# OverLordGoldDragon/ssqueezepy

Measured on AMD Instinct MI355X. Metric: ssq_cwt transforms/sec (N=160k, 300 scales, f32), higher is better.
Workload: dtype f32; 1 GPU; ssq_cwt('gmw'), N=160000, 300 log scales (nv=32), float32, two-chirp+noise; algo=blockzoom+tiles, tile_kernel=float64 tile, unordered ds_add_f64, column pair per lane (tile3_kernel)

## Files before the change

### ssqueezepy_amd/csrc/ssq_blocks.h

```cpp
#pragma once
#include "ssq_common.h"
#include "ssq_fft.h"
#include "ssq_tiles.h"
#include <algorithm>
#include <vector>

namespace ssq {

struct BlockRowDev {
    int32_t cls;
    int32_t klo;
    int32_t KP;
    int32_t L;
    int32_t G;
    int32_t pb_off;
};

struct BlockClassDev {
    int64_t P, m, V, nb;
    int64_t ctw_off;
    int64_t xb_off;
    int64_t blk_off;
    int64_t xb_stride;
    int64_t analytic;
};

struct BlockPlan {
    int64_t M = 0, N = 0, n1 = 0, na = 0, max_batch = 1;
    int dtype = SSQ_F32;
    int group = 1;
    int ncu = 256;
    int nc = 0;
    DeviceArena mem;
    std::vector<BlockClassDev> hcls;
    BlockClassDev* classes = nullptr;
    BlockRowDev* rows = nullptr;
    void* pbank = nullptr;
    void* pxi = nullptr;
    void* ctw = nullptr; void* ftw = nullptr;
    void* items[5] = {nullptr, nullptr, nullptr, nullptr, nullptr};
    std::vector<int32_t> h_items[5];
    int64_t n_items[5] = {0, 0, 0, 0, 0};
    int64_t ftw_off[5] = {0, 0, 0, 0, 0};
    void* blocks = nullptr;
    void* xb = nullptr;
    std::vector<FftPlan> ffts;
    std::vector<int> fft_first;
    void* xa = nullptr;
    FftPlan inv_m;
    AnalyticFft* ana = nullptr;
    int n_analytic = 0;
    bool own4096 = false;
    bool own_big = false;
    int64_t n_generic = 0;
    bool exact_ok = false;
    int exA = 0, exB = 0, n_exact = 0;
    void* twM = nullptr; void* zbuf = nullptr;
    const float* e_bank = nullptr; const int64_t* e_off = nullptr; const int32_t* e_lo = nullptr;
    const int32_t* e_rows = nullptr;
    int setup_exact(const float* bank_dev, const int64_t* band_off_dev, const int32_t* band_lo_dev,
                    const int32_t* gen_rows_dev, const std::vector<int64_t>& h_off,
                    const std::vector<int32_t>& h_lo, const std::vector<int32_t>& h_gen);
    int run_exact(int sig, int nsig, const void* xh_all, float* Wx, float* dWx, float* w, unsigned short* kidx,
                  const float* row_scale, double dt, const SsqParams& sp, hipStream_t stream);

    int create(const ssq_cwt_blocks_desc& d, int dtype, int64_t M, int64_t N, int64_t n1, int64_t na,
               int64_t max_batch);
    void destroy();
    int64_t bytes() const;
    int spectra(const void* xp, const void* xh, int64_t batch, hipStream_t stream,
                const unsigned char* need = nullptr);
    int run(int sig, int nsig, float* Wx, float* dWx, float* w, unsigned short* kidx,
            const float* row_scale, double dt, const SsqParams& sp, hipStream_t stream,
            const int64_t* limit = nullptr);
    int run64(int sig, int nsig, double* Wx, double* dWx, double* w, unsigned short* kidx,
              const double* row_scale, double dt, const SsqParams& sp, hipStream_t stream);
};

}
```

### ssqueezepy_amd/csrc/ssq_cwt_blocks.hip

```cpp
#include "ssq_common.h"
#include "ssq_blocks.h"
#include "ssq_ldsfft.h"
#include <cmath>

namespace ssq {

#include "ssq_point_math.inl"

struct EmitRow {
    float2* W; float2* D; float* w; unsigned short* k;
    float rs; bool scale; double gamma; int64_t omax;
    float m2hi, m2lo;
    int fx, fa;
};
__device__ __forceinline__ EmitRow make_emit_row(float* Wx, float* dWx, float* w, unsigned short* kidx,
                                                 const float* row_scale, int sig, int ksig, int row,
                                                 int64_t na, int64_t N, double gamma, int flipud) {
    EmitRow e;
    const int64_t base = ((int64_t)sig * na + row) * N;
    e.W = reinterpret_cast<float2*>(Wx) + base;
    e.D = dWx ? reinterpret_cast<float2*>(dWx) + base : nullptr;
    e.w = w ? w + base : nullptr;
    e.k = kidx ? kidx + (int64_t)ksig * na * N + kidx_index(row, 0, na, N) : nullptr;
    e.scale = row_scale != nullptr;
// ... 2 lines not shown
    const float g2 = (float)(gamma * gamma);
    e.m2hi = g2 * 1.000004f; e.m2lo = g2 * 0.999996f;
    e.fx = flipud ? -1 : 0; e.fa = flipud ? (int)na : 0;
    return e;
}
template <bool LEAN, int GRID>
__device__ __forceinline__ bool emit_point(const EmitRow& e, int j, c32 W, c32 D, const SsqParams& sp) {
    float c = W.x, d = W.y, a = D.x, b = D.y;
    if constexpr (LEAN) {
        e.W[(unsigned)j] = make_float2(c, d);
        const float m2 = c * c + d * d, num = b * c - a * d;
        const bool above = m2 > e.m2hi, below = m2 < e.m2lo;
        const float w32 = fabsf(num * __builtin_amdgcn_rcpf(m2 * 6.2831855f));
        bool ok;
        const int kb = bin_screen_cwt<GRID>(w32, sp, (int)e.omax, ok);
        const int kf = (kb ^ e.fx) + e.fa;
        e.k[(unsigned)j] = (unsigned short)(above ? kf : 0xFFFF);
        return !(below | (above & ok));
    } else {
        c = c * e.rs; d = d * e.rs; a = a * e.rs; b = b * e.rs;
        e.W[j] = make_float2(c, d);
        if (e.D) e.D[j] = make_float2(a, b);
        if (e.w) {
            float wv;
            if (mag_lt(c, d, (float)e.gamma)) wv = INFINITY;
            else wv = (float)fabs(phase_ratio(a, b, c, d));
            e.w[j] = wv;
        }
        if (e.k) {
            const int above = mag_gt_screen(c, d, e.gamma);
            if (above < 0) return true;
            unsigned short kk = 0xFFFFu;
            if (above) {
                const int kb = bin_of_point_screen(a, b, c, d, sp, (int)e.omax);
                if (kb == -2) return true;
                kk = (unsigned short)(sp.flipud ? (int)e.omax - kb : kb);
            }
            e.k[j] = kk;
        }
        return false;
    }
}
template <int V> struct GridTag { static constexpr int value = V; };
template <bool LEAN, typename F>
__device__ __forceinline__ void dispatch_grid(int grid, F&& f) {
    if constexpr (LEAN) {
        if (grid == SSQ_GRID_LOG) f(GridTag<SSQ_GRID_LOG>{});
        else if (grid == SSQ_GRID_LOG_PIECEWISE) f(GridTag<SSQ_GRID_LOG_PIECEWISE>{});
        else f(GridTag<SSQ_GRID_LIN>{});
    } else {
        f(GridTag<-1>{});
    }
}
__device__ __forceinline__ void emit_point_exact(const EmitRow& e, unsigned short* kout, c32 W, c32 D,
                                                 const SsqParams& sp) {
    const float c = W.x * e.rs, d = W.y * e.rs, a = D.x * e.rs, b = D.y * e.rs;
    unsigned short kk = 0xFFFFu;
    if (mag_of(c, d) > e.gamma) {
        const int64_t kb = bin_of_point_exact(a, b, c, d, sp, e.omax);
        kk = (unsigned short)(sp.flipud ? e.omax - kb : kb);
    }
    *kout = kk;
}
struct BlockArgs {
    const int4* items;
    const BlockRowDev* rows;
    const BlockClassDev* classes;
    const float* pbank;
    const float* pxi;
    const c32* ctw;
    const c32* ftw;
    const c32* xb;
    const float* row_scale;
    float* Wx; float* dWx; float* w; unsigned short* kidx;
    int64_t M, N, na, n_items;
    double h;
    float inv_dt;
    double gamma;
    int sig;
    bool lean() const { return kidx && !dWx && !w && !row_scale; }
    bool wx_alone() const { return !kidx && !dWx && !w; }
};

template <int L, bool LEAN, bool NOD = false>
__device__ __forceinline__ void blockzoom_body(const BlockArgs& A, const SsqParams& sp, int item_idx,
                                               c32* __restrict__ buf, c32* __restrict__ spow,
                                               c32* __restrict__ wrapf, c32* __restrict__ bandW,
                                               c32* __restrict__ bandD) {
    using S = FftShape<L>;
    constexpr int G = S::G, R1 = S::R1, RL = S::RL;
    const int tid = threadIdx.x;
    const int4 item = A.items[item_idx];
    const int row = item.x, blk = item.y, c0 = item.z;
    const BlockRowDev r = A.rows[row];
    const BlockClassDev cl = A.classes[item.w];
    const int P = (int)cl.P, Rp = P / L;
    const int sig = A.sig + (int)blockIdx.y;
    const c32* xb = A.xb + cl.xb_off + ((int64_t)sig * cl.nb + blk) * cl.xb_stride;
    const c32* ctw = A.ctw + cl.ctw_off;
    const float* psi = A.pbank + r.pb_off;
    const float* pxi = A.pxi + r.pb_off;

    constexpr bool STAGE = (L <= 512);
    const float invP = 1.0f / (float)P;
    constexpr bool EARLY = !STAGE && (R1 * G <= NT);
    float e_p[EARLY ? PPT : 1], e_m[EARLY ? PPT : 1];
    c32 e_X[EARLY ? PPT : 1], e_cw[EARLY ? PPT / R1 : 1];
    if constexpr (EARLY) {
        constexpr int NBe = PPT / R1, STR = L / R1;
        c32 st_v = {0.f, 0.f}, st_w = {0.f, 0.f};
        if (tid < R1 * G) {
            const unsigned t = (unsigned)(tid / G), col = (unsigned)(c0 + tid % G);
            st_v = ctw[(t * (unsigned)STR * col) & (unsigned)(P - 1)];
        }
        if (tid < G) st_w = ctw[(0u - (unsigned)L * (unsigned)(c0 + tid)) & (unsigned)(P - 1)];
#pragma unroll
        for (int it = 0; it < NBe; ++it) {
            const int idx = tid + it * NT, g = idx % G, u = idx / G;
            const int off0 = (u - r.klo) & (L - 1);
            e_cw[it] = ctw[((unsigned)(r.klo + off0) * (unsigned)(c0 + g)) & (unsigned)(P - 1)];
#pragma unroll
            for (int k = 0; k < R1; ++k) {
                const int off = (off0 + k * STR) & (L - 1);
                const bool in = off < r.KP;
                e_p[it * R1 + k] = in ? psi[off] : 0.f;
                e_X[it * R1 + k] = in ? xb[r.klo + off] : c32{0.f, 0.f};
                e_m[it * R1 + k] = in ? pxi[off] : 0.f;
            }
        }
        if (tid < R1 * G) spow[tid] = st_v;
        if (tid < G) wrapf[tid] = st_w;
    } else {
        constexpr int STR = L / R1;
        for (int i = tid; i < R1 * G; i += NT) {
            const unsigned t = (unsigned)(i / G), col = (unsigned)(c0 + i % G);
            spow[i] = ctw[(t * (unsigned)STR * col) & (unsigned)(P - 1)];
        }
        if (tid < G) {
            const unsigned col = (unsigned)(c0 + tid);
            wrapf[tid] = ctw[(0u - (unsigned)L * col) & (unsigned)(P - 1)];
        }
        if constexpr (STAGE) {
            for (int off = tid; off < L; off += NT) {
                c32 b = {0.f, 0.f}, d = {0.f, 0.f};
                if (off < r.KP) {
                    const float p = psi[off] * invP;
                    const c32 X = xb[r.klo + off];
                    b = {p * X.x, p * X.y};
                    const float mm = pxi[off] * A.inv_dt;
                    d = {-(b.y * mm), b.x * mm};
                }
                bandW[off] = b; bandD[off] = d;
            }
        }
    }
    __syncthreads();
    c32 zw[PPT], zd[PPT];
    {
        constexpr int NB = PPT / R1, STR = L / R1;
#pragma unroll
        for (int it = 0; it < NB; ++it) {
            const int idx = tid + it * NT, g = idx % G, u = idx / G;
            const unsigned col = (unsigned)(c0 + g);
            const int off0 = (u - r.klo) & (L - 1);
            const c32 cw0 = EARLY ? e_cw[EARLY ? it : 0] : ctw[((unsigned)(r.klo + off0) * col) & (unsigned)(P - 1)];
            const c32 wf = wrapf[g];
#pragma unroll
            for (int k = 0; k < R1; ++k) {
                const int offu = off0 + k * STR;
                const int off = offu & (L - 1);
                c32 z = {0.f, 0.f}, dz = {0.f, 0.f};
                if constexpr (STAGE) {
                    c32 cw = (k == 0) ? cw0 : cmul_v(cw0, spow[k * G + g]);
                    if (offu >= L) cw = cmul_v(cw, wf);
                    z = cmul_v(bandW[off], cw);
                    dz = cmul_v(bandD[off], cw);
                } else if (EARLY || off < r.KP) {
                    const float p = (EARLY ? e_p[EARLY ? it * R1 + k : 0] : psi[off]) * invP;
                    const c32 X = EARLY ? e_X[EARLY ? it * R1 + k : 0] : xb[r.klo + off];
                    c32 cw = (k == 0) ? cw0 : cmul_v(cw0, spow[k * G + g]);
                    if (offu >= L) cw = cmul_v(cw, wf);
                    const c32 bz = {p * X.x, p * X.y};
                    z = cmul_v(bz, cw);
                    const float mm = (EARLY ? e_m[EARLY ? it * R1 + k : 0] : pxi[off]) * A.inv_dt;
                    dz = {-(z.y * mm), z.x * mm};
                }
                zw[it * R1 + k] = z; zd[it * R1 + k] = dz;
            }
        }
    }
    lds_ifft<L, true, true>(zw, buf, A.ftw, tid);
    if constexpr (!NOD) lds_ifft<L, true>(zd, buf, A.ftw, tid);

    constexpr int NB = PPT / RL, STR = L / RL;
    const EmitRow er = make_emit_row(A.Wx, A.dWx, A.w, A.kidx, A.row_scale, sig, (int)blockIdx.y, row, A.na, A.N, A.gamma, sp.flipud);
    const int m = (int)cl.m, N = (int)A.N;
    const int jbase = blk * (int)cl.V - m + c0;
    const unsigned span = (unsigned)max(0, min((int)cl.V, N - blk * (int)cl.V));
    unsigned pend = 0;
    auto emit_all = [&](auto grid_tag) {
        constexpr int GRID = decltype(grid_tag)::value;
#pragma unroll
        for (int it = 0; it < NB; ++it) {
            const int idx = tid + it * NT, g = idx % G, u = idx / G;
#pragma unroll
            for (int k = 0; k < RL; ++k) {
                const int dcol = (u + k * STR) * Rp + g + (c0 - m);
                if ((unsigned)dcol >= span) continue;
                const int j = dcol + blk * (int)cl.V;
                if constexpr (NOD) {
                    er.W[j] = make_float2(zw[it * RL + k].x * er.rs, zw[it * RL + k].y * er.rs);
                    continue;
                }
                if (emit_point<LEAN, GRID>(er, j, zw[it * RL + k], NOD ? c32{0.f, 0.f} : zd[it * RL + k], sp))
                    pend |= 1u << (it * RL + k);
            }
        }
    };
    dispatch_grid<LEAN>(sp.grid, emit_all);
    while (__builtin_amdgcn_ballot_w64(pend != 0)) {
        const unsigned low = pend & (0u - pend);
        pend ^= low;
        c32 W = {0.f, 0.f}, D = {0.f, 0.f};
        int j = 0;
#pragma unroll
        for (int it = 0; it < NB; ++it) {
            const int idx = tid + it * NT, g = idx % G, u = idx / G;
#pragma unroll
            for (int k = 0; k < RL; ++k)
                if (low == (1u << (it * RL + k))) {
                    W = zw[it * RL + k]; D = NOD ? c32{0.f, 0.f} : zd[it * RL + k]; j = jbase + (u + k * STR) * Rp + g;
                }
        }
        if (low) emit_point_exact(er, er.k + j, W, D, sp);
    }
}

template <int L, bool LEAN, bool NOD = false>
__global__ __launch_bounds__(NT) void blockzoom_kernel(BlockArgs A, SsqParams sp) {
    __shared__ c32 buf[D_POINTS];
    __shared__ c32 spow[FftShape<L>::R1 * FftShape<L>::G];
    __shared__ c32 wrapf[FftShape<L>::G];
    __shared__ c32 bandW[(L <= 512) ? L : 1], bandD[(L <= 512) ? L : 1];
    blockzoom_body<L, LEAN, NOD>(A, sp, (int)blockIdx.x, buf, spow, wrapf, bandW, bandD);
}

struct BlockMultiArgs {
    BlockArgs A;
    const int4* items[5]; const c32* ftw[5];
    int first[6];
};
template <bool LEAN, bool NOD = false>
__global__ __launch_bounds__(NT) void blockzoom_multi_kernel(BlockMultiArgs M, SsqParams sp) {
    __shared__ c32 buf[D_POINTS];
    __shared__ c32 spow[512];
    __shared__ c32 wrapf[32];
    __shared__ c32 bandW[512], bandD[512];
    const int b = (int)blockIdx.x;
    int s = 0;
#pragma unroll
    for (int k = 1; k < 5; ++k) s += b >= M.first[k];
    BlockArgs A = M.A;
    A.items = M.items[s]; A.ftw = M.ftw[s];
    const int it = b - M.first[s];
    switch (s) {
        case 0: blockzoom_body<128, LEAN, NOD>(A, sp, it, buf, spow, wrapf, bandW, bandD); break;
        case 1: blockzoom_body<256, LEAN, NOD>(A, sp, it, buf, spow, wrapf, bandW, bandD); break;
        case 2: blockzoom_body<512, LEAN, NOD>(A, sp, it, buf, spow, wrapf, bandW, bandD); break;
        case 3: blockzoom_body<1024, LEAN, NOD>(A, sp, it, buf, spow, wrapf, bandW, bandD); break;
        default: blockzoom_body<2048, LEAN, NOD>(A, sp, it, buf, spow, wrapf, bandW, bandD); break;
    }
}

struct BlockArgs64 {
    const int4* items; const BlockRowDev* rows; const BlockClassDev* classes;
    const double* pbank; const double* pxi;
    const c64* ctw; const c64* ftw; const c64* xb;
    const double* row_scale;
    double* Wx; double* dWx; double* w; unsigned short* kidx;
    int64_t M, N, na, n_items;
    double inv_dt, gamma;
    int sig;
    bool wx_alone() const { return !kidx && !dWx && !w; }
};

template <int L, bool NOD = false>
__global__ __launch_bounds__(FftGeom<double>::NT) SSQ_WAVES_PER_EU(2, 2) void blockzoom_f64_kernel(BlockArgs64 A, SsqParams sp) {
    using S = FftShape<L, double>;
    constexpr int NT64 = FftGeom<double>::NT, G = S::G, R1 = S::R1, RL = S::RL;
    __shared__ c64 buf[FftGeom<double>::D];
    __shared__ c64 spow[R1 * G];
    __shared__ c64 wrapf[G];
    const int tid = threadIdx.x;
    const int4 item = A.items[blockIdx.x];
    const int row = item.x, blk = item.y, c0 = item.z;
    const BlockRowDev r = A.rows[row];
    const BlockClassDev cl = A.classes[item.w];
    const int P = (int)cl.P, Rp = P / L;
    const int sig = A.sig + (int)blockIdx.y;
    const c64* xb = A.xb + cl.xb_off + ((int64_t)sig * cl.nb + blk) * cl.xb_stride;
    const c64* ctw = A.ctw + cl.ctw_off;
    const double* psi = A.pbank + r.pb_off;
    const double* pxi = A.pxi + r.pb_off;
    const double invP = 1.0 / (double)P;
    constexpr int NBP = PPT / R1, STRP = L / R1;
    double bp[PPT], bm[PPT]; c64 bX[PPT];
#pragma unroll
    for (int it = 0; it < NBP; ++it) {
        const int u = (tid + it * NT64) / G;
        const int off0 = (u - r.klo) & (L - 1);
#pragma unroll
        for (int k = 0; k < R1; ++k) {
            const int off = (off0 + k * STRP) & (L - 1);
            const int oc = off < r.KP ? off : 0;
            bp[it * R1 + k] = psi[oc]; bX[it * R1 + k] = xb[r.klo + oc]; bm[it * R1 + k] = pxi[oc];
        }
    }
    {
        constexpr int STR = L / R1;
        for (int i = tid; i < R1 * G; i += NT64) {
            const unsigned t = (unsigned)(i / G), col = (unsigned)(c0 + i % G);
            spow[i] = ctw[(t * (unsigned)STR * col) & (unsigned)(P - 1)];
        }
        if (tid < G) {
            const unsigned col = (unsigned)(c0 + tid);
            wrapf[tid] = ctw[(0u - (unsigned)L * col) & (unsigned)(P - 1)];
        }
    }
    c64 cw0s[NBP];
#pragma unroll
    for (int it = 0; it < NBP; ++it) {
        const int idx = tid + it * NT64, g = idx % G, u = idx / G;
        const int off0 = (u - r.klo) & (L - 1);
        cw0s[it] = ctw[((unsigned)(r.klo + off0) * (unsigned)(c0 + g)) & (unsigned)(P - 1)];
    }
    __syncthreads();
    c64 zw[PPT], zd[PPT];
    {
        constexpr int NB = PPT / R1, STR = L / R1;
#pragma unroll
        for (int it = 0; it < NB; ++it) {
            const int idx = tid + it * NT64, g = idx % G, u = idx / G;
            const int off0 = (u - r.klo) & (L - 1);
            const c64 cw0 = cw0s[it];
            const c64 wf = wrapf[g];
#pragma unroll
            for (int k = 0; k < R1; ++k) {
                const int offu = off0 + k * STR, off = offu & (L - 1);
                const bool in = off < r.KP;
                const double p = bp[it * R1 + k] * invP;
                const c64 X = bX[it * R1 + k];
                const double mm = bm[it * R1 + k] * A.inv_dt;
                c64 cw = (k == 0) ? cw0 : cmul(cw0, spow[k * G + g]);
// ... 365 lines not shown
                                                   c32* __restrict__ stw) {
    constexpr int L = WIDE_L, P = L * C, NTH = 64 * CW, SL = CW / C;
    const int tid = threadIdx.x;
    const int g = tid % CW, u = tid / CW, slot = g / C, r = g % C;
    const int64_t sig = blockIdx.y, M = A.M;
    const bool ana = k.analytic != 0;
    const int nunits = ana ? (int)k.nb : ((int)k.nb + 1) / 2;
    const c32* __restrict__ tw = A.ctw + k.ctw_off;
    const c32* __restrict__ xa = A.xa + sig * M;
    const float* __restrict__ xp = A.xp + sig * M;
    const int64_t lead = A.n1 - k.m;
    const int m32 = (int)M;
    wide_stage_tw<CW, C>(stw, tw, tid);
    c32 w[PPT / C][C];
    wide_load_w<CW, C>(w, tw, tid);
    c32 z[PPT];
    {
        const int unit = b * SL + slot;
        const bool live = unit < nunits;
        const int b0 = ana ? unit : 2 * unit, b1 = b0 + 1;
        const bool two = !ana && b1 < (int)k.nb;
        int64_t o0 = (lead + (int64_t)b0 * k.V) % M; if (o0 < 0) o0 += M;
        int64_t o1 = (lead + (int64_t)b1 * k.V) % M; if (o1 < 0) o1 += M;
        const int a0 = (int)o0, a1 = (int)o1;
#pragma unroll
        for (int t = 0; t < PPT; ++t) {
            const int p = (u + t * (L / 16)) * C + r;
            int s0 = a0 + p; if (s0 >= m32) s0 -= m32;
            int s1 = a1 + p; if (s1 >= m32) s1 -= m32;
            c32 v = {0.f, 0.f};
            if (live) {
                if (ana) v = xa[s0];
                else v = {xp[s0], two ? xp[s1] : 0.f};
            }
            z[t] = v;
        }
    }
    wide_ifft<CW>(z, buf, stw, tid);
    wide_natural<CW, C>(z, buf, w, tid);
    for (int sl = 0; sl < SL; ++sl) {
        const int unit = b * SL + sl;
        if (unit >= nunits) break;
        const int b0 = ana ? unit : 2 * unit;
        const bool two = !ana && b0 + 1 < (int)k.nb;
        const c32* __restrict__ Y = buf + sl * P;
        c32* out0 = A.xb + k.xb_off + (sig * k.nb + b0) * k.xb_stride;
        if (ana) {
            for (int f = tid; f < P; f += NTH) out0[f] = Y[(P - f) & (P - 1)];
        } else {
            c32* out1 = out0 + k.xb_stride;
            for (int f = tid; f <= P / 2; f += NTH) {
                const c32 Pk = Y[f], Qk = Y[(P - f) & (P - 1)];
                out0[f] = {0.5f * (Qk.x + Pk.x), 0.5f * (Qk.y - Pk.y)};
                if (two) out1[f] = {0.5f * (Qk.y + Pk.y), 0.5f * (Pk.x - Qk.x)};
            }
        }
    }
}
template <int QMAX>
__global__ __launch_bounds__(NT * QMAX) void block_spectra_multi_kernel(BlockSpecArgs A) {
    __shared__ c32 buf[4096 * QMAX];
    __shared__ c32 stw[WIDE_L];
    int b = (int)blockIdx.x, c = 0;
    while (c + 1 < A.ncls && b >= A.first[c + 1]) ++c;
    b -= A.first[c];
    const BlockClassDev k = A.classes[A.cls[c]];
    if (k.P == A.M && k.nb == 1 && !k.analytic && A.xh) {
        const int64_t M = A.M, sig = blockIdx.y;
        int64_t o = (A.n1 - k.m) % M; if (o < 0) o += M;
        const c32* __restrict__ tw = A.ctw + k.ctw_off;
        const c32* __restrict__ xh = A.xh + sig * (M / 2 + 1);
        c32* __restrict__ out0 = A.xb + k.xb_off + sig * k.nb * k.xb_stride;
        const unsigned mask = (unsigned)M - 1u, ou = (unsigned)o;
        for (int f = (int)threadIdx.x; f <= (int)(M / 2); f += NT * QMAX)
            out0[f] = cmul_v(xh[f], tw[((unsigned)f * ou) & mask]);
        return;
    }
    if (k.P == 4096) block_spectra_wide<4 * QMAX, 4>(A, k, b, buf, stw);
    else if (k.P == 8192) block_spectra_wide<4 * QMAX, 8>(A, k, b, buf, stw);
    else if constexpr (QMAX >= 4) block_spectra_wide<4 * QMAX, 16>(A, k, b, buf, stw);
}

template <int L>
static int launch_zoom(const BlockArgs& A, const SsqParams& sp, int nsig, hipStream_t stream) {
    if (A.n_items == 0) return 0;
    const dim3 grid((unsigned)A.n_items, (unsigned)nsig);
    if (A.lean())
        hipLaunchKernelGGL((blockzoom_kernel<L, true>), grid, dim3(NT), 0, stream, A, sp);
    else if (A.wx_alone())
        hipLaunchKernelGGL((blockzoom_kernel<L, false, true>), grid, dim3(NT), 0, stream, A, sp);
    else
        hipLaunchKernelGGL((blockzoom_kernel<L, false>), grid, dim3(NT), 0, stream, A, sp);
    SSQ_LAUNCH_CHECK();
    return 0;
}

int BlockPlan::create(const ssq_cwt_blocks_desc& d, int dtype_, int64_t M_, int64_t N_, int64_t n1_,
                      int64_t na_, int64_t max_batch_) {
    M = M_; N = N_; n1 = n1_; na = na_; max_batch = max_batch_; dtype = dtype_;
    const size_t rs = dtype == SSQ_F32 ? 4 : 8;
    nc = d.n_classes;
    hcls.resize(nc);
    int64_t xb_total = 0, blk_max = 0;
    for (int c = 0; c < nc; ++c) {
        BlockClassDev& k = hcls[c];
        k.P = d.classes[5 * c]; k.m = d.classes[5 * c + 1]; k.V = d.classes[5 * c + 2];
        k.nb = d.classes[5 * c + 3];
        k.analytic = d.classes[5 * c + 4] ? 1 : 0;
        SSQ_REQUIRE(c == 0 || hcls[c - 1].analytic <= k.analytic, "block classes: analytic classes must come last");
        k.ctw_off = d.ctw_off[c];
        k.xb_stride = k.analytic ? k.P : k.P / 2 + 1;
        k.xb_off = xb_total;
        xb_total += max_batch * k.nb * k.xb_stride;
        k.blk_off = blk_max;
        if (!k.analytic) blk_max += max_batch * k.nb * k.P;
        n_analytic += (int)k.analytic;
    }
    int rc;
    if ((rc = mem.upload(&classes, hcls.data(), sizeof(BlockClassDev) * nc))) return rc;
    static_assert(sizeof(BlockRowDev) == 6 * sizeof(int32_t), "row table layout");
    if ((rc = mem.upload(&rows, d.rows, sizeof(BlockRowDev) * na))) return rc;
    if ((rc = mem.upload(&pbank, d.pbank, rs * d.n_pbank))) return rc;
    if ((rc = mem.upload(&pxi, d.pxi, rs * d.n_pbank))) return rc;
    if ((rc = mem.upload(&ctw, d.ctw, 2 * rs * (size_t)d.ctw_off[nc]))) return rc;
    if ((rc = mem.upload(&ftw, d.ftw, 2 * rs * (size_t)d.n_ftw))) return rc;
    for (int s = 0; s < 5; ++s) {
        n_items[s] = d.n_items[s];
        ftw_off[s] = d.ftw_off[s];
        if ((rc = mem.upload(&items[s], d.items[s], sizeof(int4) * (size_t)d.n_items[s]))) return rc;
        if (d.n_items[s]) h_items[s].assign(d.items[s], d.items[s] + 4 * d.n_items[s]);
    }
    if ((rc = mem.alloc(&xb, 2 * rs * (size_t)xb_total))) return rc;
    if ((rc = mem.alloc(&blocks, rs * (size_t)blk_max))) return rc;
    for (int c = 0; c < nc;) {
        int e = c;
        int64_t nblocks = 0;
        while (e < nc && hcls[e].P == hcls[c].P && hcls[e].analytic == hcls[c].analytic)
            nblocks += max_batch * hcls[e++].nb;
        FftPlan fp;
        rc = fp.create(hcls[c].analytic ? 2 : 0, dtype, (size_t)hcls[c].P, (size_t)nblocks, 1.0);
        if (rc) { fp.destroy(); return rc; }
        ffts.push_back(fp); fft_first.push_back(c);
        c = e;
    }
    if (n_analytic) {
        if ((rc = mem.alloc(&xa, 2 * rs * (size_t)(max_batch * M)))) return rc;
        if (AnalyticFft::supports(dtype, M)) {
            ana = new AnalyticFft();
            if ((rc = ana->create(M, max_batch))) return rc;
        } else {
            rc = inv_m.create(1, dtype, (size_t)M, (size_t)max_batch, 1.0 / (double)M);
            if (rc) return rc;
        }
    }
    n_generic = d.n_generic;
    own4096 = dtype == SSQ_F32 && M > 4096 && !(getenv("SSQ_DEBUG_BLOCK_SPECTRA") && !strcmp(getenv("SSQ_DEBUG_BLOCK_SPECTRA"), "rocfft"));
    own_big = own4096 && !(getenv("SSQ_DEBUG_BLOCK_SPECTRA") && !strcmp(getenv("SSQ_DEBUG_BLOCK_SPECTRA"), "4096"));
    {
        int dev = 0; hipDeviceProp_t pr;
        bool lds128 = false;
        if (hipGetDevice(&dev) == hipSuccess && hipGetDeviceProperties(&pr, dev) == hipSuccess && pr.multiProcessorCount > 0) {
            ncu = pr.multiProcessorCount;
            lds128 = (size_t)pr.maxSharedMemoryPerMultiProcessor >= 128 * 1024;
        }
        own_big = own_big && lds128;
    }
    return 0;
}

void BlockPlan::destroy() {
    for (auto& f : ffts) f.destroy();
    inv_m.destroy();
    if (ana) { ana->destroy(); delete ana; ana = nullptr; }
    mem.release();
}

int64_t BlockPlan::bytes() const {
    int64_t b = mem.bytes() + (int64_t)inv_m.work_bytes + (ana ? ana->mem.bytes() : 0);
    for (const FftPlan& f : ffts) b += (int64_t)f.work_bytes;
    return b;
}

int BlockPlan::spectra(const void* xp, const void* xh, int64_t batch, hipStream_t stream,
                       const unsigned char* need) {
    (void)batch;
    std::vector<char> run_on(ffts.size(), 1);
    int lo[2] = {nc, nc}, hi[2] = {-1, -1};
    bool any_analytic = false;
    BlockSpecArgs S;
    S.ncls = 0; S.first[0] = 0;
    int qmax = 1;
    bool prefix[2] = {true, true};
    for (size_t f = 0; f < ffts.size(); ++f) {
        const int a = fft_first[f], b = f + 1 < ffts.size() ? fft_first[f + 1] : nc;
        bool on = !need;
        for (int c = a; c < b && !on; ++c) on = need[c] != 0;
        const int kind = (int)hcls[a].analytic;
        any_analytic = any_analytic || (on && kind);
        int wanted = 0;
        int64_t group_wgs = 0;
        for (int c = a; c < b; ++c) {
            if (need && !need[c]) continue;
            ++wanted;
            group_wgs += kind ? hcls[c].nb : (hcls[c].nb + 1) / 2;
        }
        const int64_t Pg = hcls[a].P;
        bool whole = Pg == M && !kind && xh;
        for (int c = a; c < b && whole; ++c) whole = hcls[c].nb == 1;
        const bool small = own_big && M < ((int64_t)1 << 30) && group_wgs * max_batch <= 2 * (int64_t)ncu &&
                           (whole || ((Pg == 8192 || Pg == 16384) && Pg <= M));
        if (on && own4096 && prefix[kind] && (Pg == 4096 || small) && S.ncls + wanted <= 8) {
            for (int c = a; c < b; ++c) {
                if (need && !need[c]) continue;
                S.cls[S.ncls++] = c;
                const bool twist = Pg == M && hcls[c].nb == 1 && !kind && xh;
                qmax = std::max(qmax, twist ? 2 : (int)(Pg / 4096));
            }
            on = false;
        }
        run_on[f] = on;
        if (on) prefix[kind] = false;
        if (on) { lo[kind] = std::min(lo[kind], a); hi[kind] = std::max(hi[kind], b - 1); }
    }
    const size_t rs = dtype == SSQ_F32 ? 4 : 8;
    if (any_analytic) {
        SSQ_REQUIRE(xh && xa, "analytic block classes need the half spectrum");
        if (ana) {
            int rc = ana->run(xh, xa, max_batch, stream);
            if (rc) return rc;
        } else {
            dim3 ga((unsigned)std::min<int64_t>((max_batch * M + 255) / 256, 4096));
            int rc = dispatch_dtype(dtype, [&](auto t) {
                using C = cx<decltype(t)>;
                hipLaunchKernelGGL(analytic_spectrum_kernel<C>, ga, dim3(256), 0, stream, (const C*)xh, (C*)xa, M, max_batch);
                SSQ_LAUNCH_CHECK();
                return 0;
            });
            if (rc) return rc;
            rc = inv_m.execute(xa, nullptr, stream);
            if (rc) return rc;
        }
    }
    if (S.ncls) {
        S.xp = (const float*)xp; S.xa = (const c32*)xa; S.xb = (c32*)xb; S.xh = (const c32*)xh;
        S.classes = classes; S.ctw = (const c32*)ctw; S.M = M; S.n1 = n1;
        for (int i = 0; i < S.ncls; ++i) {
            const BlockClassDev& k = hcls[S.cls[i]];
            const int64_t units = k.analytic ? k.nb : (k.nb + 1) / 2;
            const int64_t per = std::max<int64_t>(1, qmax / (k.P / 4096));
            S.first[i + 1] = S.first[i] + (int)((units + per - 1) / per);
        }
        const dim3 sg((unsigned)S.first[S.ncls], (unsigned)max_batch);
        if (qmax == 1)
            hipLaunchKernelGGL(block_spectra4096_kernel, sg, dim3(NT), 0, stream, S);
        else if (qmax == 2)
            hipLaunchKernelGGL(block_spectra_multi_kernel<2>, sg, dim3(NT * 2), 0, stream, S);
        else
            hipLaunchKernelGGL(block_spectra_multi_kernel<4>, sg, dim3(NT * 4), 0, stream, S);
        SSQ_LAUNCH_CHECK();
    }
    for (int kind = 0; kind < 2; ++kind) {
        if (hi[kind] < lo[kind]) continue;
        int64_t most = 0;
        for (int c = lo[kind]; c <= hi[kind]; ++c) most = std::max<int64_t>(most, max_batch * hcls[c].nb * hcls[c].P);
        dim3 grid((unsigned)std::min<int64_t>((most + 255) / 256, 2048), (unsigned)(hi[kind] - lo[kind] + 1));
        const int rc = dispatch_dtype(dtype, [&](auto t) {
            using T = decltype(t);
            using C = cx<T>;
            if (kind == 0)
                hipLaunchKernelGGL((gather_blocks_kernel<T, false>), grid, dim3(256), 0, stream, (const T*)xp,
                                   (T*)blocks, classes + lo[0], M, n1, max_batch);
            else
                hipLaunchKernelGGL((gather_blocks_kernel<C, true>), grid, dim3(256), 0, stream, (const C*)xa,
                                   (C*)xb, classes + lo[1], M, n1, max_batch);
            SSQ_LAUNCH_CHECK();
            return 0;
        });
        if (rc) return rc;
    }
    for (size_t f = 0; f < ffts.size(); ++f) {
        if (!run_on[f]) continue;
        const BlockClassDev& k = hcls[fft_first[f]];
        int rc = k.analytic ? ffts[f].execute((char*)xb + (size_t)k.xb_off * 2 * rs, nullptr, stream)
                            : ffts[f].execute((char*)blocks + (size_t)k.blk_off * rs,
                                              (char*)xb + (size_t)k.xb_off * 2 * rs, stream);
        if (rc) return rc;
    }
    return 0;
}

int BlockPlan::run(int sig, int nsig, float* Wx, float* dWx, float* w, unsigned short* kidx,
                   const float* row_scale, double dt, const SsqParams& sp, hipStream_t stream,
                   const int64_t* limit) {
    BlockArgs A;
    A.rows = rows; A.classes = classes; A.pbank = (const float*)pbank; A.pxi = (const float*)pxi;
    A.ctw = (const c32*)ctw;
    A.xb = (const c32*)xb; A.row_scale = row_scale;
    A.Wx = Wx; A.dWx = dWx; A.w = w; A.kidx = kidx;
    A.M = M; A.N = N; A.na = na;
    A.h = (2.0 * 3.141592653589793) / (double)M;
    A.inv_dt = 1.0f / (float)dt;
    A.gamma = sp.gamma; A.sig = sig;
    {
        const char* fe = getenv("SSQ_DEBUG_CWT_BLOCKS_MULTI");
        const int force = fe ? atoi(fe) : -1;
        int64_t total = 0, biggest = 0; int used = 0;
        for (int s = 0; s < 5; ++s) {
            const int64_t n = limit ? limit[s] : n_items[s];
            total += n; biggest = std::max(biggest, n * nsig); used += n > 0;
        }
        const bool lean = A.lean();
        const bool multi = force >= 0 ? force != 0
                                      : (used > 1 && (lean || biggest <= 2 * (int64_t)ncu || total * nsig <= 18 * (int64_t)ncu));
        if (multi && total > 0) {
            BlockMultiArgs Mx;
            Mx.A = A; Mx.A.items = nullptr; Mx.A.n_items = total; Mx.A.ftw = nullptr;
            int acc = 0;
            for (int s = 0; s < 5; ++s) {
                Mx.items[s] = (const int4*)items[s]; Mx.ftw[s] = (const c32*)ftw + ftw_off[s];
                Mx.first[s] = acc; acc += (int)(limit ? limit[s] : n_items[s]);
            }
            Mx.first[5] = acc;
            const dim3 grid((unsigned)total, (unsigned)nsig);
            if (lean)
                hipLaunchKernelGGL((blockzoom_multi_kernel<true>), grid, dim3(NT), 0, stream, Mx, sp);
            else if (A.wx_alone())
                hipLaunchKernelGGL((blockzoom_multi_kernel<false, true>), grid, dim3(NT), 0, stream, Mx, sp);
            else
                hipLaunchKernelGGL((blockzoom_multi_kernel<false>), grid, dim3(NT), 0, stream, Mx, sp);
            SSQ_LAUNCH_CHECK();
            return 0;
        }
    }
    for (int s = 0; s < 5; ++s) {
        A.items = (const int4*)items[s]; A.n_items = limit ? limit[s] : n_items[s];
        A.ftw = (const c32*)ftw + ftw_off[s];
        const int rc = fft_dispatch<128, 2048>(128 << s, [&](auto len) { return launch_zoom<decltype(len)::value>(A, sp, nsig, stream); });
        if (rc) return rc;
    }
    return 0;
}


int BlockPlan::setup_exact(const float* bank_dev, const int64_t* band_off_dev, const int32_t* band_lo_dev,
                           const int32_t* gen_rows_dev, const std::vector<int64_t>& h_off,
                           const std::vector<int32_t>& h_lo, const std::vector<int32_t>& h_gen) {
    exact_ok = false;
    if (h_gen.empty()) return 0;
    const int lm = fft_slot(M, 1);
    if ((1ll << lm) != M || lm < 14 || lm > 22) return 0;
    for (int32_t i : h_gen) {
        int64_t len = h_off[i + 1] - h_off[i];
        if (h_lo[i] + len > M / 2 + 1) return 0;
    }
    exA = 1 << ((lm + 1) / 2); exB = (int)(M / exA);
    e_bank = bank_dev; e_off = band_off_dev; e_lo = band_lo_dev; e_rows = gen_rows_dev;
    n_exact = (int)h_gen.size();
    std::vector<float> tw((size_t)2 * M);
    for (int64_t q = 0; q < M; ++q) {
        double ang = 2.0 * 3.14159265358979323846 * (double)q / (double)M;
        tw[2 * q] = (float)(cos(ang) / (double)M); tw[2 * q + 1] = (float)(sin(ang) / (double)M);
    }
    int rc;
    if ((rc = mem.upload(&twM, tw.data(), 8 * (size_t)M))) return rc;
    if ((rc = mem.alloc(&zbuf, (size_t)group * n_exact * 2 * M * 8))) return rc;
    exact_ok = true;
    return 0;
}

template <int L>
static int launch_exact1(const ExactArgs& E, int n_rows, int nsig, hipStream_t stream) {
    hipLaunchKernelGGL((exact_pass1_kernel<L>), dim3((unsigned)(E.A / FftShape<L>::G), (unsigned)n_rows, (unsigned)nsig),
                       dim3(NT), 0, stream, E);
    SSQ_LAUNCH_CHECK();
    return 0;
}
template <int L>
static int launch_exact2(const ExactArgs& E, const SsqParams& sp, int n_rows, int nsig, hipStream_t stream) {
    const dim3 grid((unsigned)(E.B / FftShape<L>::G), (unsigned)n_rows, (unsigned)nsig);
    if (E.lean())
        hipLaunchKernelGGL((exact_pass2_kernel<L, true>), grid, dim3(NT), 0, stream, E, sp);
    else
        hipLaunchKernelGGL((exact_pass2_kernel<L, false>), grid, dim3(NT), 0, stream, E, sp);
    SSQ_LAUNCH_CHECK();
    return 0;
}

int BlockPlan::run_exact(int sig, int nsig, const void* xh_all, float* Wx, float* dWx, float* w,
                         unsigned short* kidx, const float* row_scale, double dt, const SsqParams& sp,
                         hipStream_t stream) {
    ExactArgs E;
    E.bank = e_bank; E.band_off = e_off; E.band_lo = e_lo; E.rows = e_rows;
    E.xh = (const c32*)xh_all; E.Z = (c32*)zbuf; E.twM = (const c32*)twM; E.row_scale = row_scale;
    E.Wx = Wx; E.dWx = dWx; E.w = w; E.kidx = kidx;
    E.M = M; E.N = N; E.na = na; E.A = exA; E.B = exB; E.n1pad = (int)n1; E.sig = sig; E.n_rows = n_exact;
    E.G2 = D_POINTS / exA;
    E.h = (2.0 * 3.141592653589793) / (double)M; E.inv_dt = 1.0f / (float)dt; E.gamma = sp.gamma;
    const int rc = fft_dispatch<128, 2048>(exB, [&](auto len) {
        E.ftw = (const c32*)ftw + ftw_off[fft_slot(decltype(len)::value, 128)];
        return launch_exact1<decltype(len)::value>(E, n_exact, nsig, stream);
    });
    if (rc) return rc;
    return fft_dispatch<128, 2048>(exA, [&](auto len) {
        E.ftw = (const c32*)ftw + ftw_off[fft_slot(decltype(len)::value, 128)];
        return launch_exact2<decltype(len)::value>(E, sp, n_exact, nsig, stream);
    });
}

}
```

### ssqueezepy_amd/csrc/ssq_ldsfft.h

```cpp
#pragma once
#include <hip/hip_runtime.h>
#include "ssq_common.h"
#include <cmath>
#include <vector>

namespace ssq {

template <typename R> struct cx { R x, y; };
using c32 = cx<float>;
using c64 = cx<double>;

__device__ __forceinline__ float fma_(float a, float b, float c) { return __builtin_fmaf(a, b, c); }
__device__ __forceinline__ double fma_(double a, double b, double c) { return __builtin_fma(a, b, c); }

template <typename R> __device__ __forceinline__ cx<R> cmul(cx<R> a, cx<R> b) {
    return {fma_(a.x, b.x, -(a.y * b.y)), fma_(a.x, b.y, a.y * b.x)};
}
__device__ __forceinline__ cx<float> cmul_v(cx<float> a, cx<float> b) {
    ssq_f2 av, bv, dv;
    av.x = a.x; av.y = a.y; bv.x = b.x; bv.y = b.y;
    SSQ_CMUL_PK(dv, av, bv);
    return {dv.x, dv.y};
}
__device__ __forceinline__ cx<double> cmul_v(cx<double> a, cx<double> b) { return cmul(a, b); }
template <typename R> __device__ __forceinline__ cx<R> cadd(cx<R> a, cx<R> b) { return {a.x + b.x, a.y + b.y}; }
template <typename R> __device__ __forceinline__ cx<R> csub(cx<R> a, cx<R> b) { return {a.x - b.x, a.y - b.y}; }
template <typename R> __device__ __forceinline__ cx<R> mul_i(cx<R> a) { return {-a.y, a.x}; }

template <typename R> __device__ __forceinline__ void dft2(cx<R>& a, cx<R>& b) { cx<R> t = a; a = cadd(t, b); b = csub(t, b); }

template <typename R>
__device__ __forceinline__ void dft4(cx<R>& v0, cx<R>& v1, cx<R>& v2, cx<R>& v3) {
    cx<R> a = cadd(v0, v2), b = csub(v0, v2), c = cadd(v1, v3), d = mul_i(csub(v1, v3));
    v0 = cadd(a, c); v1 = cadd(b, d); v2 = csub(a, c); v3 = csub(b, d);
}

template <int R> struct Dft;
template <> struct Dft<4> {
    template <typename R> static __device__ __forceinline__ void run(cx<R> (&v)[4]) { dft4(v[0], v[1], v[2], v[3]); }
};
template <> struct Dft<8> {
    template <typename R> static __device__ __forceinline__ void run(cx<R> (&v)[8]) {
        cx<R> e[4] = {v[0], v[2], v[4], v[6]}, o[4] = {v[1], v[3], v[5], v[7]};
        dft4(e[0], e[1], e[2], e[3]);
        dft4(o[0], o[1], o[2], o[3]);
        const R h = (R)0.70710678118654752440;
        o[1] = {h * (o[1].x - o[1].y), h * (o[1].x + o[1].y)};
        o[2] = mul_i(o[2]);
        o[3] = {-h * (o[3].x + o[3].y), h * (o[3].x - o[3].y)};
#pragma unroll
        for (int k = 0; k < 4; ++k) { v[k] = cadd(e[k], o[k]); v[k + 4] = csub(e[k], o[k]); }
    }
};
template <> struct Dft<16> {
    template <typename R> static __device__ __forceinline__ void run(cx<R> (&v)[16]) {
        const R c1 = (R)0.92387953251128675613, s1 = (R)0.38268343236508977173;
        const R h = (R)0.70710678118654752440;
        cx<R> a[4][4];
#pragma unroll
        for (int t1 = 0; t1 < 4; ++t1) {
            a[t1][0] = v[t1]; a[t1][1] = v[t1 + 4]; a[t1][2] = v[t1 + 8]; a[t1][3] = v[t1 + 12];
            dft4(a[t1][0], a[t1][1], a[t1][2], a[t1][3]);
        }
        const cx<R> w[10] = {{1, 0}, {c1, s1}, {h, h}, {s1, c1}, {0, 1}, {-s1, c1}, {-h, h}, {-c1, s1},
                           {-1, 0}, {-c1, -s1}};
#pragma unroll
        for (int t1 = 1; t1 < 4; ++t1)
#pragma unroll
            for (int k2 = 1; k2 < 4; ++k2) a[t1][k2] = cmul(a[t1][k2], w[t1 * k2]);
#pragma unroll
        for (int k2 = 0; k2 < 4; ++k2) {
            cx<R> b0 = a[0][k2], b1 = a[1][k2], b2 = a[2][k2], b3 = a[3][k2];
            dft4(b0, b1, b2, b3);
            v[k2] = b0; v[k2 + 4] = b1; v[k2 + 8] = b2; v[k2 + 12] = b3;
        }
    }
};

constexpr int PPT = 16;
template <typename R> struct FftGeom {
    static constexpr int NT = sizeof(R) == 4 ? 256 : 128;
    static constexpr int D = NT * PPT;
};
constexpr int D_POINTS = FftGeom<float>::D;
constexpr int NT = FftGeom<float>::NT;

// ... 56 lines not shown
    constexpr bool three = (R3 > 1);
    constexpr bool ETW = EARLY_TW && sizeof(R) == 4;
    if constexpr (!FRESH) __syncthreads();
    {
        constexpr int NB = PPT / R1;
#pragma unroll
        for (int it = 0; it < NB; ++it) {
            cx<R> t[R1];
#pragma unroll
            for (int k = 0; k < R1; ++k) t[k] = v[it * R1 + k];
            Dft<R1>::run(t);
            int idx = tid + it * NT, g = idx % G, u = idx / G;
#pragma unroll
            for (int k = 0; k < R1; ++k) buf[(u * R1 + k) * G + g] = t[k];
        }
    }
    cx<R> tw2[ETW ? PPT / R2 : 1][ETW ? R2 : 1];
    if constexpr (ETW) {
        constexpr int NB = PPT / R2, Ns = R1, TW = L / (Ns * R2);
#pragma unroll
        for (int it = 0; it < NB; ++it) {
            const int kk = ((tid + it * NT) / G) % Ns;
#pragma unroll
            for (int k = 1; k < R2; ++k) tw2[it][k] = ftw[kk * k * TW * TWS];
        }
    }
    __syncthreads();
    {
        constexpr int NB = PPT / R2, Ns = R1, STR = L / R2;
        cx<R> t[NB][R2];
#pragma unroll
        for (int it = 0; it < NB; ++it) {
            int idx = tid + it * NT, g = idx % G, u = idx / G;
#pragma unroll
            for (int k = 0; k < R2; ++k) t[it][k] = buf[(u + k * STR) * G + g];
        }
        if (three) __syncthreads();
#pragma unroll
        for (int it = 0; it < NB; ++it) {
            int idx = tid + it * NT, g = idx % G, u = idx / G;
            int kk = u % Ns;
            constexpr int TW = L / (Ns * R2);
#pragma unroll
            for (int k = 1; k < R2; ++k) t[it][k] = cmul_v(t[it][k], ETW ? tw2[ETW ? it : 0][ETW ? k : 0] : ftw[kk * k * TW * TWS]);
            Dft<R2>::run(t[it]);
            if (three) {
                int j0 = (u / Ns) * Ns * R2 + kk;
#pragma unroll
                for (int k = 0; k < R2; ++k) buf[(j0 + k * Ns) * G + g] = t[it][k];
            } else {
#pragma unroll
                for (int k = 0; k < R2; ++k) v[it * R2 + k] = t[it][k];
            }
        }
    }
    if constexpr (three) {
        cx<R> tw3[ETW ? PPT / R3 : 1][ETW ? R3 : 1];
        if constexpr (ETW) {
#pragma unroll
            for (int it = 0; it < PPT / R3; ++it) {
                const int kk = ((tid + it * NT) / G) % (R1 * R2);
#pragma unroll
                for (int k = 1; k < R3; ++k) tw3[it][k] = ftw[kk * k * TWS];
            }
        }
        __syncthreads();
        constexpr int NB = PPT / R3, Ns = R1 * R2, STR = L / R3;
#pragma unroll
        for (int it = 0; it < NB; ++it) {
            int idx = tid + it * NT, g = idx % G, u = idx / G;
            cx<R> t[R3];
#pragma unroll
            for (int k = 0; k < R3; ++k) t[k] = buf[(u + k * STR) * G + g];
            int kk = u % Ns;
#pragma unroll
            for (int k = 1; k < R3; ++k) t[k] = cmul_v(t[k], ETW ? tw3[ETW ? it : 0][ETW ? k : 0] : ftw[kk * k * TWS]);
            Dft<R3>::run(t);
#pragma unroll
            for (int k = 0; k < R3; ++k) v[it * R3 + k] = t[k];
        }
    }
}

}
```

Before: 3761 transforms/s.

## Interleave the Wx and dWx inverse LDS FFTs in the blockzoom kernels

Adds lds_ifft2, which runs the two inverse FFTs for Wx and dWx together in one shared LDS buffer. The butterflies of one transform are staggered between the LDS transpose passes of the other, and the twiddle loads are hoisted. The LDS layout gets padding to reduce bank conflicts. This is meant to hide LDS latency and barrier stalls by overlapping the ALU work of one transform with the exchange of the other. The cost is higher register pressure from holding both arrays plus twiddles, and a somewhat larger shared buffer. An environment variable can turn it off, and wx-alone dispatch now takes priority over lean.

Result: faster. 3871 transforms/s, median of 6 (+2.9%).

```diff
diff --git a/ssqueezepy_amd/csrc/ssq_blocks.h b/ssqueezepy_amd/csrc/ssq_blocks.h
--- a/ssqueezepy_amd/csrc/ssq_blocks.h
+++ b/ssqueezepy_amd/csrc/ssq_blocks.h
@@ -52,6 +52,7 @@
     int n_analytic = 0;
     bool own4096 = false;
     bool own_big = false;
+    bool paired = true;
     int64_t n_generic = 0;
     bool exact_ok = false;
     int exA = 0, exB = 0, n_exact = 0;
diff --git a/ssqueezepy_amd/csrc/ssq_cwt_blocks.hip b/ssqueezepy_amd/csrc/ssq_cwt_blocks.hip
--- a/ssqueezepy_amd/csrc/ssq_cwt_blocks.hip
+++ b/ssqueezepy_amd/csrc/ssq_cwt_blocks.hip
@@ -108,7 +108,7 @@
     bool wx_alone() const { return !kidx && !dWx && !w; }
 };
 
-template <int L, bool LEAN, bool NOD = false>
+template <int L, bool LEAN, bool NOD = false, bool PAIRED = true>
 __device__ __forceinline__ void blockzoom_body(const BlockArgs& A, const SsqParams& sp, int item_idx,
                                                c32* __restrict__ buf, c32* __restrict__ spow,
                                                c32* __restrict__ wrapf, c32* __restrict__ bandW,
@@ -215,8 +215,12 @@
             }
         }
     }
-    lds_ifft<L, true, true>(zw, buf, A.ftw, tid);
-    if constexpr (!NOD) lds_ifft<L, true>(zd, buf, A.ftw, tid);
+    if constexpr (PAIRED && !NOD) {
+        lds_ifft2<L>(zw, zd, buf, A.ftw, tid);
+    } else {
+        lds_ifft<L, true, true>(zw, buf, A.ftw, tid);
+        if constexpr (!NOD) lds_ifft<L, true>(zd, buf, A.ftw, tid);
+    }
 
     constexpr int NB = PPT / RL, STR = L / RL;
     const EmitRow er = make_emit_row(A.Wx, A.dWx, A.w, A.kidx, A.row_scale, sig, (int)blockIdx.y, row, A.na, A.N, A.gamma, sp.flipud);
@@ -262,13 +266,13 @@
     }
 }
 
-template <int L, bool LEAN, bool NOD = false>
+template <int L, bool LEAN, bool NOD = false, bool PAIRED = true>
 __global__ __launch_bounds__(NT) void blockzoom_kernel(BlockArgs A, SsqParams sp) {
-    __shared__ c32 buf[D_POINTS];
+    __shared__ c32 buf[(PAIRED && !NOD) ? lds_ifft2_points<L> : D_POINTS];
     __shared__ c32 spow[FftShape<L>::R1 * FftShape<L>::G];
     __shared__ c32 wrapf[FftShape<L>::G];
     __shared__ c32 bandW[(L <= 512) ? L : 1], bandD[(L <= 512) ? L : 1];
-    blockzoom_body<L, LEAN, NOD>(A, sp, (int)blockIdx.x, buf, spow, wrapf, bandW, bandD);
+    blockzoom_body<L, LEAN, NOD, PAIRED>(A, sp, (int)blockIdx.x, buf, spow, wrapf, bandW, bandD);
 }
 
 struct BlockMultiArgs {
@@ -276,9 +280,9 @@
     const int4* items[5]; const c32* ftw[5];
     int first[6];
 };
-template <bool LEAN, bool NOD = false>
+template <bool LEAN, bool NOD = false, bool PAIRED = true>
 __global__ __launch_bounds__(NT) void blockzoom_multi_kernel(BlockMultiArgs M, SsqParams sp) {
-    __shared__ c32 buf[D_POINTS];
+    __shared__ c32 buf[(PAIRED && !NOD) ? lds_ifft2_points<2048> : D_POINTS];
     __shared__ c32 spow[512];
     __shared__ c32 wrapf[32];
     __shared__ c32 bandW[512], bandD[512];
@@ -290,11 +294,11 @@
     A.items = M.items[s]; A.ftw = M.ftw[s];
     const int it = b - M.first[s];
     switch (s) {
-        case 0: blockzoom_body<128, LEAN, NOD>(A, sp, it, buf, spow, wrapf, bandW, bandD); break;
-        case 1: blockzoom_body<256, LEAN, NOD>(A, sp, it, buf, spow, wrapf, bandW, bandD); break;
-        case 2: blockzoom_body<512, LEAN, NOD>(A, sp, it, buf, spow, wrapf, bandW, bandD); break;
-        case 3: blockzoom_body<1024, LEAN, NOD>(A, sp, it, buf, spow, wrapf, bandW, bandD); break;
-        default: blockzoom_body<2048, LEAN, NOD>(A, sp, it, buf, spow, wrapf, bandW, bandD); break;
+        case 0: blockzoom_body<128, LEAN, NOD, PAIRED>(A, sp, it, buf, spow, wrapf, bandW, bandD); break;
+        case 1: blockzoom_body<256, LEAN, NOD, PAIRED>(A, sp, it, buf, spow, wrapf, bandW, bandD); break;
+        case 2: blockzoom_body<512, LEAN, NOD, PAIRED>(A, sp, it, buf, spow, wrapf, bandW, bandD); break;
+        case 3: blockzoom_body<1024, LEAN, NOD, PAIRED>(A, sp, it, buf, spow, wrapf, bandW, bandD); break;
+        default: blockzoom_body<2048, LEAN, NOD, PAIRED>(A, sp, it, buf, spow, wrapf, bandW, bandD); break;
     }
 }
 
@@ -826,15 +830,19 @@
 }
 
 template <int L>
-static int launch_zoom(const BlockArgs& A, const SsqParams& sp, int nsig, hipStream_t stream) {
+static int launch_zoom(const BlockArgs& A, const SsqParams& sp, int nsig, bool paired, hipStream_t stream) {
     if (A.n_items == 0) return 0;
     const dim3 grid((unsigned)A.n_items, (unsigned)nsig);
-    if (A.lean())
+    if (A.wx_alone())
+        hipLaunchKernelGGL((blockzoom_kernel<L, false, true>), grid, dim3(NT), 0, stream, A, sp);
+    else if (A.lean() && paired)
         hipLaunchKernelGGL((blockzoom_kernel<L, true>), grid, dim3(NT), 0, stream, A, sp);
-    else if (A.wx_alone())
-        hipLaunchKernelGGL((blockzoom_kernel<L, false, true>), grid, dim3(NT), 0, stream, A, sp);
+    else if (A.lean())
+        hipLaunchKernelGGL((blockzoom_kernel<L, true, false, false>), grid, dim3(NT), 0, stream, A, sp);
+    else if (paired)
+        hipLaunchKernelGGL((blockzoom_kernel<L, false>), grid, dim3(NT), 0, stream, A, sp);
     else
-        hipLaunchKernelGGL((blockzoom_kernel<L, false>), grid, dim3(NT), 0, stream, A, sp);
+        hipLaunchKernelGGL((blockzoom_kernel<L, false, false, false>), grid, dim3(NT), 0, stream, A, sp);
     SSQ_LAUNCH_CHECK();
     return 0;
 }
@@ -900,6 +908,7 @@
     n_generic = d.n_generic;
     own4096 = dtype == SSQ_F32 && M > 4096 && !(getenv("SSQ_DEBUG_BLOCK_SPECTRA") && !strcmp(getenv("SSQ_DEBUG_BLOCK_SPECTRA"), "rocfft"));
     own_big = own4096 && !(getenv("SSQ_DEBUG_BLOCK_SPECTRA") && !strcmp(getenv("SSQ_DEBUG_BLOCK_SPECTRA"), "4096"));
+    paired = !(getenv("SSQ_DEBUG_BLOCK_PAIRED") && atoi(getenv("SSQ_DEBUG_BLOCK_PAIRED")) == 0);
     {
         int dev = 0; hipDeviceProp_t pr;
         bool lds128 = false;
@@ -1066,12 +1075,16 @@
             }
             Mx.first[5] = acc;
             const dim3 grid((unsigned)total, (unsigned)nsig);
-            if (lean)
+            if (A.wx_alone())
+                hipLaunchKernelGGL((blockzoom_multi_kernel<false, true>), grid, dim3(NT), 0, stream, Mx, sp);
+            else if (lean && paired)
                 hipLaunchKernelGGL((blockzoom_multi_kernel<true>), grid, dim3(NT), 0, stream, Mx, sp);
-            else if (A.wx_alone())
-                hipLaunchKernelGGL((blockzoom_multi_kernel<false, true>), grid, dim3(NT), 0, stream, Mx, sp);
+            else if (lean)
+                hipLaunchKernelGGL((blockzoom_multi_kernel<true, false, false>), grid, dim3(NT), 0, stream, Mx, sp);
+            else if (paired)
+                hipLaunchKernelGGL((blockzoom_multi_kernel<false>), grid, dim3(NT), 0, stream, Mx, sp);
             else
-                hipLaunchKernelGGL((blockzoom_multi_kernel<false>), grid, dim3(NT), 0, stream, Mx, sp);
+                hipLaunchKernelGGL((blockzoom_multi_kernel<false, false, false>), grid, dim3(NT), 0, stream, Mx, sp);
             SSQ_LAUNCH_CHECK();
             return 0;
         }
@@ -1079,7 +1092,7 @@
     for (int s = 0; s < 5; ++s) {
         A.items = (const int4*)items[s]; A.n_items = limit ? limit[s] : n_items[s];
         A.ftw = (const c32*)ftw + ftw_off[s];
-        const int rc = fft_dispatch<128, 2048>(128 << s, [&](auto len) { return launch_zoom<decltype(len)::value>(A, sp, nsig, stream); });
+        const int rc = fft_dispatch<128, 2048>(128 << s, [&](auto len) { return launch_zoom<decltype(len)::value>(A, sp, nsig, paired, stream); });
         if (rc) return rc;
     }
     return 0;
diff --git a/ssqueezepy_amd/csrc/ssq_ldsfft.h b/ssqueezepy_amd/csrc/ssq_ldsfft.h
--- a/ssqueezepy_amd/csrc/ssq_ldsfft.h
+++ b/ssqueezepy_amd/csrc/ssq_ldsfft.h
@@ -2,6 +2,7 @@
 #include <hip/hip_runtime.h>
 #include "ssq_common.h"
 #include <cmath>
+#include <type_traits>
 #include <vector>
 
 namespace ssq {
@@ -224,4 +225,116 @@
     }
 }
 
-}
+constexpr int lds_ifft2_pad(int L) { return (FftGeom<float>::D / L <= 8) ? 2 : 0; }
+template <int L> constexpr int lds_ifft2_points = FftGeom<float>::D + lds_ifft2_pad(L) * (FftGeom<float>::D / 32);
+template <int L>
+__device__ __forceinline__ void lds_ifft2(cx<float> (&vw)[PPT], cx<float> (&vd)[PPT], cx<float>* __restrict__ buf,
+                                          const cx<float>* __restrict__ ftw, int tid) {
+    using C = cx<float>;
+    constexpr int NT = FftGeom<float>::NT, G = NT * PPT / L;
+    constexpr int R1 = FftShape<L>::R1, R2 = FftShape<L>::R2, R3 = FftShape<L>::R3;
+    constexpr bool three = (R3 > 1);
+    constexpr int NB1 = PPT / R1, NB2 = PPT / R2, STR2 = L / R2;
+    constexpr int PADE = lds_ifft2_pad(L);
+    static_assert(L >= 128 && (R1 * G) % 32 == 0 && 32 % (G < 32 ? G : 32) == 0, "lds_ifft2: strides and the padding");
+    auto slot = [](int i) { return i + PADE * (i >> 5); };
+#define SSQ_PADDED(o) ((o) + PADE * ((o) >> 5))
+    auto butterflies = [](auto rr, C (&v)[PPT], auto* tw) {
+        constexpr int RR = decltype(rr)::value;
+#pragma unroll
+        for (int it = 0; it < PPT / RR; ++it) {
+            C t[RR];
+            t[0] = v[it * RR];
+#pragma unroll
+            for (int k = 1; k < RR; ++k) {
+                if constexpr (std::is_same_v<decltype(tw), std::nullptr_t*>) t[k] = v[it * RR + k];
+                else t[k] = cmul_v(v[it * RR + k], tw[it][k]);
+            }
+            Dft<RR>::run(t);
+#pragma unroll
+            for (int k = 0; k < RR; ++k) v[it * RR + k] = t[k];
+        }
+    };
+    constexpr std::nullptr_t* none = nullptr;
+    int w1[NB1], r2[NB2];
+#pragma unroll
+    for (int it = 0; it < NB1; ++it) { const int idx = tid + it * NT; w1[it] = slot((idx / G) * R1 * G + idx % G); }
+#pragma unroll
+    for (int it = 0; it < NB2; ++it) { const int idx = tid + it * NT; r2[it] = slot(idx); }
+    auto put1 = [&](const C (&v)[PPT]) {
+#pragma unroll
+        for (int it = 0; it < NB1; ++it)
+#pragma unroll
+            for (int k = 0; k < R1; ++k) buf[w1[it] + SSQ_PADDED(k * G)] = v[it * R1 + k];
+    };
+    auto get2 = [&](C (&v)[PPT]) {
+#pragma unroll
+        for (int it = 0; it < NB2; ++it)
+#pragma unroll
+            for (int k = 0; k < R2; ++k) v[it * R2 + k] = buf[r2[it] + SSQ_PADDED(k * STR2 * G)];
+    };
+    butterflies(FftLen<R1>{}, vw, none);
+    put1(vw);
+    C tw2[NB2][R2];
+#pragma unroll
+    for (int it = 0; it < NB2; ++it) {
+        const int kk = ((tid + it * NT) / G) % R1;
+        constexpr int TW = L / (R1 * R2);
+#pragma unroll
+        for (int k = 1; k < R2; ++k) tw2[it][k] = ftw[kk * k * TW];
+    }
+    butterflies(FftLen<R1>{}, vd, none);
+    __syncthreads();
+    get2(vw);
+    __syncthreads();
+    put1(vd);
+    butterflies(FftLen<R2>{}, vw, tw2);
+    __syncthreads();
+    get2(vd);
+    if constexpr (!three) {
+        butterflies(FftLen<R2>{}, vd, tw2);
+    } else {
+        constexpr int NB3 = PPT / R3, STR3 = L / R3;
+        int w2[NB2], r3[NB3];
+#pragma unroll
+        for (int it = 0; it < NB2; ++it) {
+            const int idx = tid + it * NT, g = idx % G, u = idx / G;
+            w2[it] = slot(((u / R1) * R1 * R2 + u % R1) * G + g);
+        }
+#pragma unroll
+        for (int it = 0; it < NB3; ++it) { const int idx = tid + it * NT; r3[it] = slot(idx); }
+        auto put2 = [&](const C (&v)[PPT]) {
+#pragma unroll
+            for (int it = 0; it < NB2; ++it)
+#pragma unroll
+                for (int k = 0; k < R2; ++k) buf[w2[it] + SSQ_PADDED(k * R1 * G)] = v[it * R2 + k];
+        };
+        auto get3 = [&](C (&v)[PPT]) {
+#pragma unroll
+            for (int it = 0; it < NB3; ++it)
+#pragma unroll
+                for (int k = 0; k < R3; ++k) v[it * R3 + k] = buf[r3[it] + SSQ_PADDED(k * STR3 * G)];
+        };
+        __syncthreads();
+        put2(vw);
+        butterflies(FftLen<R2>{}, vd, tw2);
+        C tw3[NB3][R3];
+#pragma unroll
+        for (int it = 0; it < NB3; ++it) {
+            const int kk = ((tid + it * NT) / G) % (R1 * R2);
+#pragma unroll
+            for (int k = 1; k < R3; ++k) tw3[it][k] = ftw[kk * k];
+        }
+        __syncthreads();
+        get3(vw);
+        __syncthreads();
+        put2(vd);
+        butterflies(FftLen<R3>{}, vw, tw3);
+        __syncthreads();
+        get3(vd);
+        butterflies(FftLen<R3>{}, vd, tw3);
+    }
+#undef SSQ_PADDED
+}
+
+}
```
